# GrokImageCompression/Grok

Hardware: AMD Instinct MI355X
Metric: encode Mpixels/s (whole node), 8K RGB HTJ2K lossless (higher is better)
Workload: dtype int16x2 packed (exact: range-proven on the host, int32 fallback); 1 GPU; 8192x8192x3 8-bit RGB, 1 tile, RCT+5/3 lossless HTJ2K, 5 levels, 64x64 blocks (BASELINE metric shape); tiles_per_gpu=1, code_blocks_per_gpu=49152, packed_dwt_levels=4, generator=G2 (SURVEY.md §8d), parallelism=1 GPU, consecutive encodes pipelined (grk_amd_set_pipelining), prewarm_steps=40, input_frames_in_rotation=3

## Files before the change

### grok_amd/csrc/kernels_ht.hip

```cpp
#include <atomic>
#include <mutex>
#include "kernels.h"
#include "ht_common.h"
#include "ht_vlc_tables.h"
#define GRK_K3_STORE(p, v) __builtin_nontemporal_store((uint32_t)(v), (p))
#include <type_traits>

namespace grk_amd {

namespace {

typedef unsigned short u16x2 __attribute__((ext_vector_type(2)));
typedef int i32x2 __attribute__((ext_vector_type(2)));
typedef short i16x2 __attribute__((ext_vector_type(2)));

__device__ uint32_t g_vlc_enc[4096];
__device__ uint2 g_uvlc[64];

struct MelState {
    int run, k, acc, left;
    uint32_t pos;
    uint32_t word;
    uint32_t vec;
};
extern "C" __device__ int grk_amd_writelane(int value, int lane_select, int old) __asm("llvm.amdgcn.writelane.i32");
__device__ __forceinline__ void mel_writelane(uint32_t& vec, uint32_t word, uint32_t lane_index)
{
    vec = (uint32_t)grk_amd_writelane(__builtin_amdgcn_readfirstlane((int)word), __builtin_amdgcn_readfirstlane((int)lane_index), (int)vec);
}
struct MelPacked { uint32_t st, word, vec; uint64_t q; uint32_t qn; };
__device__ __forceinline__ void mel_drain(MelState& m, uint64_t q, uint32_t qn);
__device__ __forceinline__ MelState mel_unpack(const MelPacked& p)
{
    const uint32_t st = (uint32_t)__builtin_amdgcn_readfirstlane((int)p.st);
    MelState m;
    m.run = (int)(st & 63u); m.k = (int)((st >> 6) & 15u); m.acc = (int)((st >> 10) & 255u); m.left = (int)((st >> 18) & 15u);
    m.pos = st >> 22; m.word = (uint32_t)__builtin_amdgcn_readfirstlane((int)p.word); m.vec = p.vec;
    const uint64_t q = ((uint64_t)(uint32_t)__builtin_amdgcn_readfirstlane((int)(uint32_t)(p.q >> 32)) << 32) |
                       (uint32_t)__builtin_amdgcn_readfirstlane((int)(uint32_t)p.q);
    mel_drain(m, q, (uint32_t)__builtin_amdgcn_readfirstlane((int)p.qn));
    return m;
}
__device__ __forceinline__ void mel_pack(MelPacked& p, const MelState& m)
{
    p.st = (uint32_t)m.run | ((uint32_t)m.k << 6) | (((uint32_t)m.acc & 255u) << 10) | ((uint32_t)m.left << 18) | (m.pos << 22);
    p.word = m.word; p.vec = m.vec; p.q = 0; p.qn = 0;
}
__device__ __forceinline__ void mel_put_byte(MelState& m, uint32_t byte)
{
    if (m.pos < 252) {
        m.word |= byte << (8u * (m.pos & 3u));
        if ((m.pos & 3u) == 3u) { mel_writelane(m.vec, m.word, m.pos >> 2); m.word = 0; }
    }
    m.pos++;
}
__device__ __forceinline__ void mel_put_bit(MelState& m, uint8_t*, int v, bool)
{
    m.acc = (m.acc << 1) | v;
    if (--m.left == 0) {
        mel_put_byte(m, (uint32_t)m.acc & 0xFFu);
        m.left = (m.acc == 0xFF) ? 7 : 8;
        m.acc = 0;
    }
}
__device__ __forceinline__ void mel_put_bits(MelState& m, uint32_t v, uint32_t n)
{
    if ((int)n < m.left) { m.acc = (m.acc << n) | (int)v; m.left -= (int)n; return; }
    const uint32_t rem = n - (uint32_t)m.left;
    const uint32_t byte = (((uint32_t)m.acc << m.left) | (v >> rem)) & 0xFFu;
    mel_put_byte(m, byte);
    m.left = (byte == 0xFFu ? 7 : 8) - (int)rem;
    m.acc = (int)(v & ((1u << rem) - 1u));
}
__device__ __forceinline__ void mel_flush(MelState& m, uint8_t* buf, int lane)
{
    if (m.pos < 252 && (m.pos & 3u)) mel_writelane(m.vec, m.word, m.pos >> 2);
    reinterpret_cast<uint32_t*>(buf)[lane] = m.vec;
}

__device__ __forceinline__ void mel_event(MelState& m, uint8_t* buf, int one, bool writer)
{
    const int e = (int)((kMelE >> (4 * m.k)) & 0xF);
    if (!one) {
        if (++m.run >= (1 << e)) {
            mel_put_bit(m, buf, 1, writer);
            m.run = 0;
            if (m.k < 12) m.k++;
        }
    } else {
        mel_put_bits(m, (uint32_t)m.run, (uint32_t)e + 1u);
        m.run = 0;
        if (m.k > 0) m.k--;
    }
}

__device__ __forceinline__ void mel_drain(MelState& m, uint64_t q, uint32_t qn)
{
    while ((int)qn >= m.left) {
        qn -= (uint32_t)m.left;
        const uint32_t byte = (((uint32_t)m.acc << m.left) | ((uint32_t)(q >> qn) & ((1u << m.left) - 1u))) & 0xFFu;
        mel_put_byte(m, byte);
        m.left = byte == 0xFFu ? 7 : 8;
        m.acc = 0;
    }
    m.acc = (int)(((uint32_t)m.acc << qn) | ((uint32_t)q & ((1u << qn) - 1u)));
    m.left -= (int)qn;
}
__device__ __forceinline__ void mel_drain_packed(uint32_t& st, MelPacked& p, uint64_t& q, uint32_t& qn)
{
    MelState m;
    m.run = 0; m.k = 0; m.acc = (int)((st >> 10) & 255u); m.left = (int)((st >> 18) & 15u);
    m.pos = st >> 22; m.word = (uint32_t)__builtin_amdgcn_readfirstlane((int)p.word); m.vec = p.vec;
    mel_drain(m, q, qn);
    st = (st & 0x3FFu) | (((uint32_t)m.acc & 255u) << 10) | ((uint32_t)m.left << 18) | (m.pos << 22);
    p.word = m.word; p.vec = m.vec;
    q = 0; qn = 0;
}
__device__ __forceinline__ void mel_zeros(uint32_t& run, uint32_t& k4, uint64_t& q, uint32_t& qn, uint32_t nz)
{
    while (true) {
        const uint32_t need = (1u << ((uint32_t)(kMelE >> k4) & 0xFu)) - run;
        if (nz < need) { run += nz; break; }
        q = (q << 1) | 1u; qn += 1u;
        run = 0; k4 = min(k4 + 4u, 48u); nz -= need;
    }
}
__device__ __forceinline__ void mel_first_row(MelPacked& p, uint64_t EH, uint64_t EV)
{
    uint32_t run = 0, k4 = 0, qn = 0;
    uint64_t q = 0;
    if (!(EH & EV)) mel_zeros(run, k4, q, qn, (uint32_t)__builtin_popcountll(EH));
    else while (EH) {
        uint32_t e = (uint32_t)(kMelE >> k4) & 0xFu;
        uint32_t n, v, at, t0, t1, t2;
        asm volatile("s_ff1_i32_b64 %[at], %[EH]\n\t"
                     "s_bitset0_b64 %[EH], %[at]\n\t"
                     "s_add_i32 %[t1], %[run], 1\n\t"
                     "s_lshr_b32 %[t0], %[t1], %[e]\n\t"
                     "s_add_i32 %[t2], %[t0], -1\n\t"
                     "s_and_b32 %[t1], %[t1], %[t2]\n\t"
                     "s_lshl2_add_u32 %[t2], %[t0], %[k4]\n\t"
                     "s_min_i32 %[t2], %[t2], 48\n\t"
                     "s_add_i32 %[k4], %[k4], -4\n\t"
                     "s_max_i32 %[k4], %[k4], 0\n\t"
                     "s_add_i32 %[e], %[e], 1\n\t"
                     "s_bitcmp1_b64 %[EV], %[at]\n\t"
                     "s_cselect_b32 %[n], %[e], %[t0]\n\t"
                     "s_cselect_b32 %[v], %[run], %[t0]\n\t"
                     "s_cselect_b32 %[run], 0, %[t1]\n\t"
                     "s_cselect_b32 %[k4], %[k4], %[t2]"
                     : [EH] "+s"(EH), [run] "+s"(run), [k4] "+s"(k4), [e] "+s"(e), [n] "=&s"(n), [v] "=&s"(v), [at] "=&s"(at),
                       [t0] "=&s"(t0), [t1] "=&s"(t1), [t2] "=&s"(t2)
                     : [EV] "s"(EV)
                     : "scc");
        q = (q << n) | v; qn += n;
    }
    p.st = (p.st & ~0x3FFu) | run | (k4 << 4);
    p.q = q; p.qn = qn;
}

__device__ __forceinline__ void mel_row(MelPacked& p, uint64_t H, uint64_t V)
{
    uint32_t st = (uint32_t)__builtin_amdgcn_readfirstlane((int)p.st);
    uint32_t run = st & 63u, k4 = (st >> 4) & 0x3Cu;
    uint64_t q = ((uint64_t)(uint32_t)__builtin_amdgcn_readfirstlane((int)(uint32_t)(p.q >> 32)) << 32) |
                 (uint32_t)__builtin_amdgcn_readfirstlane((int)(uint32_t)p.q);
    uint32_t qn = (uint32_t)__builtin_amdgcn_readfirstlane((int)p.qn);
    if (__builtin_expect(qn > 40u, 0)) mel_drain_packed(st, p, q, qn);
    uint64_t ones = H & V;
    while (ones) {
        const uint32_t first = (uint32_t)__builtin_ctzll(ones);
        const uint64_t from = ~0ull << first;
        const uint32_t nz = (uint32_t)__builtin_popcountll(H & ~from);
        H &= from << 1; ones &= from << 1;
        uint32_t e = (uint32_t)(kMelE >> k4) & 0xFu;
        if (__builtin_expect(run + nz >= (1u << e), 0)) { mel_zeros(run, k4, q, qn, nz); e = (uint32_t)(kMelE >> k4) & 0xFu; }
        else run += nz;
        q = (q << (e + 1u)) | run; qn += e + 1u;
        run = 0; k4 = (uint32_t)max((int)k4 - 4, 0);
        if (__builtin_expect(qn > 40u, 0)) mel_drain_packed(st, p, q, qn);
    }
    if (H) mel_zeros(run, k4, q, qn, (uint32_t)__builtin_popcountll(H));
    p.st = (st & ~0x3FFu) | run | (k4 << 4);
    p.q = q; p.qn = qn;
}

__device__ __forceinline__ void mel_zero_run(MelState& m, uint8_t* buf, uint32_t n, bool writer)
{
    while (n) {
        const uint32_t need = (1u << ((kMelE >> (4 * m.k)) & 0xF)) - (uint32_t)m.run;
        if (n < need) { m.run += (int)n; return; }
        mel_put_bit(m, buf, 1, writer);
        m.run = 0;
        if (m.k < 12) m.k++;
        n -= need;
    }
}

__device__ __forceinline__ void or3_now(uint32_t& acc, uint32_t a, uint32_t b)
{
    asm("v_bitop3_b32 %0, %1, %2, %3 bitop3:0xfe" : "=v"(acc) : "v"(acc), "v"(a), "v"(b));
}
__device__ __forceinline__ void lds_or(uint32_t* p, uint32_t v)
{
    (void)__hip_atomic_fetch_or(p, v, __ATOMIC_RELAXED, __HIP_MEMORY_SCOPE_WORKGROUP);
}
__device__ __forceinline__ void or_bits64(uint32_t* raw, uint32_t pos, uint64_t val, uint32_t nbits)
{
    const uint32_t sh = pos & 31;
    uint32_t* w = raw + (pos >> 5);
    const uint64_t lo = val << sh;
    lds_or(w, (uint32_t)lo);
    lds_or(w + 1, (uint32_t)(lo >> 32));
    if (__ballot(sh + nbits > 64u)) lds_or(w + 2, ((uint32_t)(val >> 32) >> 1) >> (31 - sh));
}
__device__ __forceinline__ void or_bits32(uint32_t* raw, uint32_t pos, uint32_t val)
{
    const uint32_t sh = pos & 31;
    uint32_t* w = raw + (pos >> 5);
    const uint64_t lo = (uint64_t)val << sh;
    lds_or(w, (uint32_t)lo);
    lds_or(w + 1, (uint32_t)(lo >> 32));
}
__device__ __forceinline__ uint32_t get_bits(const uint32_t* raw, uint32_t pos, uint32_t n)
{
    const uint32_t w = pos >> 5, sh = pos & 31;
    uint64_t v = raw[w] | ((uint64_t)raw[w + 1] << 32);
    return (uint32_t)(v >> sh) & ((1u << n) - 1);
}

__device__ __forceinline__ uint32_t ffbh_i32(uint32_t t)
{
    uint32_t r;
    asm("v_ffbh_i32 %0, %1" : "=v"(r) : "v"(t));
    return r;
}

__device__ __forceinline__ uint32_t ffbh_u32(uint32_t t)
{
    uint32_t r;
    asm("v_ffbh_u32 %0, %1" : "=v"(r) : "v"(t));
    return r;
}
template <int B, int HALF>
__device__ __forceinline__ void ffbh_u16_to_byte(uint32_t& acc, uint32_t packed)
{
    if constexpr (B == 0) {
        if constexpr (HALF == 0) asm("v_ffbh_u32_sdwa %0, %1 dst_sel:BYTE_0 dst_unused:UNUSED_PAD src0_sel:WORD_0" : "=v"(acc) : "v"(packed));
        else asm("v_ffbh_u32_sdwa %0, %1 dst_sel:BYTE_0 dst_unused:UNUSED_PAD src0_sel:WORD_1" : "=v"(acc) : "v"(packed));
    } else if constexpr (B == 1) {
        if constexpr (HALF == 0) asm("v_ffbh_u32_sdwa %0, %1 dst_sel:BYTE_1 dst_unused:UNUSED_PRESERVE src0_sel:WORD_0" : "+v"(acc) : "v"(packed));
        else asm("v_ffbh_u32_sdwa %0, %1 dst_sel:BYTE_1 dst_unused:UNUSED_PRESERVE src0_sel:WORD_1" : "+v"(acc) : "v"(packed));
    } else if constexpr (B == 2) {
        if constexpr (HALF == 0) asm("v_ffbh_u32_sdwa %0, %1 dst_sel:BYTE_2 dst_unused:UNUSED_PRESERVE src0_sel:WORD_0" : "+v"(acc) : "v"(packed));
        else asm("v_ffbh_u32_sdwa %0, %1 dst_sel:BYTE_2 dst_unused:UNUSED_PRESERVE src0_sel:WORD_1" : "+v"(acc) : "v"(packed));
    } else {
        if constexpr (HALF == 0) asm("v_ffbh_u32_sdwa %0, %1 dst_sel:BYTE_3 dst_unused:UNUSED_PRESERVE src0_sel:WORD_0" : "+v"(acc) : "v"(packed));
        else asm("v_ffbh_u32_sdwa %0, %1 dst_sel:BYTE_3 dst_unused:UNUSED_PRESERVE src0_sel:WORD_1" : "+v"(acc) : "v"(packed));
    }
}
template <int B>
__device__ __forceinline__ void ffbh_i32_to_byte(uint32_t& acc, uint32_t t)
{
    if constexpr (B == 0) asm("v_ffbh_i32_sdwa %0, %1 dst_sel:BYTE_0 dst_unused:UNUSED_PAD src0_sel:DWORD" : "=v"(acc) : "v"(t));
    else if constexpr (B == 1) asm("v_ffbh_i32_sdwa %0, %1 dst_sel:BYTE_1 dst_unused:UNUSED_PRESERVE src0_sel:DWORD" : "+v"(acc) : "v"(t));
    else if constexpr (B == 2) asm("v_ffbh_i32_sdwa %0, %1 dst_sel:BYTE_2 dst_unused:UNUSED_PRESERVE src0_sel:DWORD" : "+v"(acc) : "v"(t));
    else asm("v_ffbh_i32_sdwa %0, %1 dst_sel:BYTE_3 dst_unused:UNUSED_PRESERVE src0_sel:DWORD" : "+v"(acc) : "v"(t));
}
__device__ __forceinline__ uint32_t min_of_bytes(uint32_t c)
{
    uint32_t m1, m2;
    asm("v_min_u32_sdwa %0, %1, %1 dst_sel:DWORD dst_unused:UNUSED_PAD src0_sel:BYTE_0 src1_sel:BYTE_1" : "=v"(m1) : "v"(c));
    asm("v_min_u32_sdwa %0, %1, %1 dst_sel:DWORD dst_unused:UNUSED_PAD src0_sel:BYTE_2 src1_sel:BYTE_3" : "=v"(m2) : "v"(c));
    return min(m1, m2);
}
template <int TT>
__device__ __forceinline__ uint32_t bitop3(uint32_t a, uint32_t b, uint32_t c)
{
    return (uint32_t)__builtin_amdgcn_bitop3_b32((int)a, (int)b, (int)c, TT);
}
__device__ __forceinline__ uint32_t pk_min_u16(uint32_t a, uint32_t b)
{
    uint32_t r;
    asm("v_pk_min_u16 %0, %1, %2" : "=v"(r) : "v"(a), "s"(b));
    return r;
}
__device__ __forceinline__ uint32_t pk_lshr15_u16(uint32_t a)
{
    uint32_t r;
    asm("v_pk_lshrrev_b16 %0, 15, %1 op_sel_hi:[0,1]" : "=v"(r) : "v"(a));
    return r;
}
__device__ __forceinline__ uint32_t pk_sub_u16(uint32_t a, uint32_t b)
{
    uint32_t r;
    asm("v_pk_sub_u16 %0, %1, %2" : "=v"(r) : "v"(a), "v"(b));
    return r;
}
__device__ __forceinline__ uint32_t sign_mask(uint32_t a)
{
    uint32_t r;
    asm("v_ashrrev_i32 %0, 31, %1" : "=v"(r) : "v"(a));
    return r;
}
__device__ __forceinline__ uint32_t pk_mul_lo_u16(uint32_t a, uint32_t b)
{
    uint32_t r;
// ... 311 lines not shown
            stage1(it + 2, sE, n2); stage2(it + 1, sO);
            stage1(it + 3, sO, n3); stage2(it + 2, sE);
            stage1(it + 4, sE, n0); stage2(it + 3, sO);
        }
        stage1(it + 1, sO, n1); stage2(it, sE);
        stage1(it + 2, sE, n2); stage2(it + 1, sO);
        stage1(it + 3, sO, n3); stage2(it + 2, sE);
        stage1_last(it + 4, sE, n0); stage2(it + 3, sO);
        stage1_last(it + 5, sO, n1); stage2(it + 4, sE);
        stage1_last(it + 6, sE, n2); stage2(it + 5, sO);
        stage1_last(it + 7, sO, n3); stage2(it + 6, sE);
        stage2(it + 7, sO);
    } else {
        for (uint32_t it = 0; it < itn; it += 4) {
            if (it + 1 < itn) stage1(it + 1, sO, n1);
            stage2(it, sE);
            if (it + 1 < itn) { if (it + 2 < itn) stage1(it + 2, sE, n2); stage2(it + 1, sO); }
            if (it + 2 < itn) { if (it + 3 < itn) stage1(it + 3, sO, n3); stage2(it + 2, sE); }
            if (it + 3 < itn) { if (it + 4 < itn) stage1(it + 4, sE, n0); stage2(it + 3, sO); }
        }
        asm volatile("" : : "v"(n0[0]), "v"(n0[1]), "v"(n0[2]), "v"(n0[3]), "v"(n1[0]), "v"(n1[1]), "v"(n1[2]), "v"(n1[3]),
                            "v"(n2[0]), "v"(n2[1]), "v"(n2[2]), "v"(n2[3]), "v"(n3[0]), "v"(n3[1]), "v"(n3[2]), "v"(n3[3]));
    }
    };

    auto phase_a2 = [&]() {
        constexpr bool PK = H16;
        constexpr int NW = PK ? 4 : 8;
        const uint32_t rr = (uint32_t)lane >> 4, cc = (uint32_t)lane & 15u;
        const uint32_t c0m = cc == 0 ? 0xFFFFFFFFu : 0u, c15m = cc == 15 ? 0xFFFFFFFFu : 0u;
        const uint32_t oddm = (rr & 1u) ? 0xFFFFFFFFu : 0u, row0m = rr == 0 ? 0xFFFFFFFFu : 0u;
        const uint32_t lane_off2 = 2u * rr * stride_b + 4u * cc * EB;
        typedef int i32x4 __attribute__((ext_vector_type(4)));

        auto fetch2 = [&](uint32_t it, int32_t (&r)[NW]) {
            const uint32_t o0 = lane_off2 + it * (8u * stride_b), o1 = o0 + stride_b;
            if constexpr (PK) {
                const i32x2 q0 = __builtin_nontemporal_load(reinterpret_cast<const i32x2*>(srcb + o0));
                const i32x2 q1 = __builtin_nontemporal_load(reinterpret_cast<const i32x2*>(srcb + o1));
                r[0] = q0.x; r[1] = q1.x; r[2] = q0.y; r[3] = q1.y;
            } else {
                const i32x4 q0 = __builtin_nontemporal_load(reinterpret_cast<const i32x4*>(srcb + o0));
                const i32x4 q1 = __builtin_nontemporal_load(reinterpret_cast<const i32x4*>(srcb + o1));
                r[0] = q0.x; r[2] = q0.y; r[1] = q1.x; r[3] = q1.y;
                r[4] = q0.z; r[6] = q0.w; r[5] = q1.z; r[7] = q1.w;
            }
        };
        int32_t n0[NW], n1[NW], n2[NW], n3[NW];
        fetch2(0, n0); fetch2(1, n1); fetch2(2, n2); fetch2(3, n3);

        struct Stage1 {
            uint32_t vv[2][PK ? 2 : 4];
            uint32_t SM[2], U[2], u[2], tuple[2];
            uint2 ue[2];
            uint64_t H[2], V[2];
        };
        uint32_t Aprev = 0xFFFFFFFFu;

        auto analyse = [&](const int32_t* sm, uint32_t (&vv)[PK ? 2 : 4], uint32_t& C) {
            if constexpr (PK) {
                const int32_t nw0 = sm[0], nw1 = sm[1];
                const i16x2 w0 = __builtin_bit_cast(i16x2, nw0), w1 = __builtin_bit_cast(i16x2, nw1);
                const u16x2 p0 = __builtin_bit_cast(u16x2, __builtin_elementwise_max(w0, -w0));
                const u16x2 p1 = __builtin_bit_cast(u16x2, __builtin_elementwise_max(w1, -w1));
                or3_now(ovf, __builtin_bit_cast(uint32_t, p0), __builtin_bit_cast(uint32_t, p1));
                const u16x2 one2 = {1, 1};
                const uint32_t t0 = __builtin_bit_cast(uint32_t, __builtin_elementwise_sub_sat(p0 + p0, one2));
                const uint32_t t1 = __builtin_bit_cast(uint32_t, __builtin_elementwise_sub_sat(p1 + p1, one2));
                ffbh_u16_to_byte<0, 0>(C, t0); ffbh_u16_to_byte<1, 0>(C, t1);
                ffbh_u16_to_byte<2, 1>(C, t0); ffbh_u16_to_byte<3, 1>(C, t1);
                vv[0] = pk_sub_u16(t0, pk_lshr15_u16(~(uint32_t)nw0));
                vv[1] = pk_sub_u16(t1, pk_lshr15_u16(~(uint32_t)nw1));
            } else {
                uint32_t t[4];
#pragma unroll
                for (int i = 0; i < 4; ++i) {
                    uint32_t mag;
                    if constexpr (IRREV) {
                        const float cf = __int_as_float(sm[i]);
                        const float q = __fmul_rn(fabsf(cf), inv_step);
                        mag = min((uint32_t)q, lim);
                    } else {
                        mag = (uint32_t)max(sm[i], -sm[i]);
                    }
                    ovf |= mag;
                    t[i] = (mag << 1) - 1u;
                    vv[i] = t[i] - 1u + ((uint32_t)sm[i] >> 31);
                }
                ffbh_i32_to_byte<0>(C, t[0]); ffbh_i32_to_byte<1>(C, t[1]);
                ffbh_i32_to_byte<2>(C, t[2]); ffbh_i32_to_byte<3>(C, t[3]);
            }
        };

        auto stage1r = [&](uint32_t it, Stage1& o, int32_t (&nbuf)[NW], auto refill_c) {
            uint32_t C[2];
            analyse(nbuf, o.vv[0], C[0]);
            analyse(nbuf + NW / 2, o.vv[1], C[1]);
            uint32_t N[2], rho[2], rho2[2], cm[2], emax[2];
#pragma unroll
            for (int q = 0; q < 2; ++q) {
                N[q] = bitop3<0x30>(0x01010101u, C[q] >> 7, 0u);
                rho[q] = __builtin_amdgcn_udot4(N[q], 0x08040201u, 0u, false);
                rho2[q] = __builtin_amdgcn_udot4(N[q], 0x20100804u, 0u, false);
                cm[q] = min_of_bytes(C[q]);
                emax[q] = 32u - min(cm[q], 32u);
            }
            const uint32_t Bp = __builtin_amdgcn_perm(C[1], C[0], 0x07050301u);
            const auto s16 = __builtin_amdgcn_permlane16_swap(Bp, Bp, false, false);
            const uint32_t A1 = (uint32_t)s16[1];
            const auto s32 = __builtin_amdgcn_permlane32_swap(Aprev, A1, false, false);
            const uint32_t tsel = bitop3<0xE4>((uint32_t)s32[1], (uint32_t)s32[0], row0m);
            const uint32_t Y = bitop3<0xE4>((uint32_t)s16[0], tsel, oddm);
            Aprev = A1;
            const uint32_t Yl = dpp0<0x138, 0xF>(Y) | c0m;
            const uint32_t Yr = dpp0<0x130, 0xF>(Y) | c15m;
            const uint32_t rhoBl = dpp0<0x138, 0xF>(rho[1]) & ~c0m;
            const uint32_t W[2] = {__builtin_amdgcn_alignbit(Y, Yl, 24), __builtin_amdgcn_alignbit(Yr, Y, 8)};
            const uint32_t rl[2] = {rhoBl, rho[0]};
            bool cq0[2];
#pragma unroll
            for (int q = 0; q < 2; ++q) {
                const uint32_t m4 = min_of_bytes(W[q]);
                const int kap_e = 31 - (int)m4;
                const uint32_t gmask = sign_mask(0xFEE80000u << (15u - rho[q]));
                const uint32_t kappa = (uint32_t)max(1, kap_e & (int)gmask);
                const uint32_t F = W[q] & (W[q] >> 8);
                uint32_t coff = bitop3<0xEA>(F << 3, 0x400u, 0x2000u);
                coff = bitop3<0xEA>(F >> 11, 0x1000u, coff);
                coff = bitop3<0xEA>((rl[q] & 0xCu) + 0x7FCu, 0x800u, coff);
                cq0[q] = (coff & 0x1C00u) == 0x1400u;
                if (it == 0) {
                    const uint32_t cq_first = (rl[q] >> 1) | (rl[q] & 1u);
                    coff = rr ? coff : cq_first << 10;
                    cq0[q] = rr ? cq0[q] : cq_first == 0u;
                }
                const uint32_t U = max(emax[q], kappa);
                const uint32_t u = U - kappa;
                const uint32_t X = C[q] - __builtin_amdgcn_perm(cm[q], cm[q], 0u);
                const uint32_t Yz = (X & 0x1F1F1F1Fu) + 0x7F7F7F7Fu;
                const uint32_t e4 = __builtin_amdgcn_udot4(bitop3<0x30>(0x01010101u, Yz >> 7, 0u), 0x20100804u, 0u, false);
                const uint32_t um = sign_mask(0u - u);
                const uint32_t off = ((rho2[q] << 4) | coff) | bitop3<0x80>(e4, rho2[q], um);
                o.tuple[q] = *reinterpret_cast<const uint32_t*>(vtab + off);
                o.SM[q] = N[q] * 255u; o.U[q] = U; o.u[q] = u;
                if (it != 0) o.ue[q] = uvlc_l[u];
            }
            o.H[0] = __ballot(cq0[0]); o.V[0] = o.H[0] & __ballot(rho[0] != 0);
            o.H[1] = __ballot(cq0[1]); o.V[1] = o.H[1] & __ballot(rho[1] != 0);
            if constexpr (decltype(refill_c)::value) {
                __builtin_amdgcn_sched_barrier(0);
                fetch2(it + 4u, nbuf);
            }
        };
        auto stage1 = [&](uint32_t it, Stage1& o, int32_t (&nbuf)[NW]) { stage1r(it, o, nbuf, std::true_type{}); };
        auto stage1_last = [&](uint32_t it, Stage1& o, int32_t (&nbuf)[NW]) { stage1r(it, o, nbuf, std::false_type{}); };

        auto stage2 = [&](uint32_t it, const Stage1& s) {
            uint32_t vm[2][4], M4[2], m1[2], m2[2], m3[2], m01[2], m23[2], qlen[2];
#pragma unroll
            for (int q = 0; q < 2; ++q) {
                M4[q] = (__builtin_amdgcn_perm(s.U[q], s.U[q], 0u) - (s.tuple[q] & 0x01010101u)) & s.SM[q];
                qlen[q] = __builtin_amdgcn_udot4(M4[q], 0x01010101u, 0u, false);
                m01[q] = __builtin_amdgcn_udot4(M4[q], 0x00000101u, 0u, false);
                m23[q] = qlen[q] - m01[q];
                m1[q] = M4[q] >> 8; m2[q] = M4[q] >> 16; m3[q] = M4[q] >> 24;
                if constexpr (PK) {
                    vm[q][0] = __builtin_amdgcn_ubfe(s.vv[q][0], 0u, M4[q]); vm[q][2] = __builtin_amdgcn_ubfe(s.vv[q][0], 16u, m2[q]);
                    vm[q][1] = __builtin_amdgcn_ubfe(s.vv[q][1], 0u, m1[q]); vm[q][3] = __builtin_amdgcn_ubfe(s.vv[q][1], 16u, m3[q]);
                } else {
                    vm[q][0] = __builtin_amdgcn_ubfe(s.vv[q][0], 0u, M4[q]); vm[q][2] = __builtin_amdgcn_ubfe(s.vv[q][2], 0u, m2[q]);
                    vm[q][1] = __builtin_amdgcn_ubfe(s.vv[q][1], 0u, m1[q]); vm[q][3] = __builtin_amdgcn_ubfe(s.vv[q][3], 0u, m3[q]);
                }
            }
            const uint32_t ms_len = qlen[0] + qlen[1];

            uint32_t uiA = s.u[0], uiB = s.u[1];
            bool xev = false, xv = false;
            if (it == 0) {
                const bool first = rr == 0;
                const uint32_t uA = s.u[0], uB = s.u[1];
                const bool both = first && uA > 2 && uB > 2;
                uiA = both ? uA - 2 : uA;
                uiB = both ? uB - 2 : uB;
                uiB = (first && uA > 2 && uB > 0 && uB <= 2) ? 32u + uB : uiB;
                xev = first && uA > 0 && uB > 0;
                xv = xev && min(uA, uB) > 2;
            }
            const uint2 ueA = it == 0 ? uvlc_l[uiA] : s.ue[0], ueB = it == 0 ? uvlc_l[uiB] : s.ue[1];
            const uint32_t AA = (s.tuple[0] >> 25) | ueA.x, AB = (s.tuple[1] >> 25) | ueB.x;
            const uint32_t LA = ((s.tuple[0] >> 4) & 7u) | ueA.y, LB = ((s.tuple[1] >> 4) & 7u) | ueB.y;
            const uint32_t S = LA + LB;
            const uint32_t lenA = LA & 0xFFu, slen = S & 0xFFu;
            const uint32_t o_preB = slen + ((LA >> 8) & 0xFFu);
            const uint32_t o_sufA = slen + ((S >> 8) & 0xFFu);
            const uint32_t o_sufB = o_sufA + (LA >> 16);
            const uint32_t cl = o_sufA + (S >> 16);
            const uint32_t wv = (AA & 0xFFu) | ((AB & 0xFFu) << lenA) | (((AA >> 8) & 0xFFu) << slen) | (((AB >> 8) & 0xFFu) << o_preB) |
                                ((AA >> 16) << o_sufA) | ((AB >> 16) << o_sufB);

            const uint32_t packed = ms_len | (cl << 16);
            const uint32_t incl = wave_incl_scan(packed);
            const uint32_t tot = (uint32_t)__builtin_amdgcn_readlane((int)incl, 63);
            const uint32_t mpos = ms_bits + ((incl - packed) & 0xFFFFu);
            const uint32_t vpos = vlc_bits + (incl >> 16) - cl;
            ms_bits += tot & 0xFFFFu;
            vlc_bits += tot >> 16;
            if (((L.ms_cap_bits - ms_bits) | (L.vlc_cap_bits - vlc_bits)) >> 31) { lds_full = true; return; }

            if (ms_len != 0u) {
                if (!__ballot(max(qlen[0], qlen[1]) > 32u)) {
                    const uint32_t qa = (vm[0][0] | (vm[0][1] << (M4[0] & 31u))) | ((vm[0][2] | (vm[0][3] << (m2[0] & 31u))) << (m01[0] & 31u));
                    const uint32_t qb = (vm[1][0] | (vm[1][1] << (M4[1] & 31u))) | ((vm[1][2] | (vm[1][3] << (m2[1] & 31u))) << (m01[1] & 31u));
                    or_bits64(ms_raw, mpos, (uint64_t)qa | ((uint64_t)qb << qlen[0]), ms_len);
                } else {
#pragma unroll
                    for (int q = 0; q < 2; ++q) {
                        const uint32_t at = q ? mpos + qlen[0] : mpos;
                        if (narrow || !__ballot(max(m01[q], m23[q]) > 32u)) {
                            const uint32_t v01 = vm[q][0] | (vm[q][1] << (M4[q] & 31u));
                            const uint32_t v23 = vm[q][2] | (vm[q][3] << (m2[q] & 31u));
                            or_bits64(ms_raw, at, (uint64_t)v01 | ((uint64_t)v23 << m01[q]), qlen[q]);
                        } else {
                            or_bits64(ms_raw, at, (uint64_t)vm[q][0] | ((uint64_t)vm[q][1] << (M4[q] & 0xFFu)), m01[q]);
                            or_bits64(ms_raw, at + m01[q], (uint64_t)vm[q][2] | ((uint64_t)vm[q][3] << (m2[q] & 0xFFu)), m23[q]);
                        }
                    }
                }
            }
            if (cl != 0u) or_bits32(vlc_raw, vpos, wv);

            uint64_t HA = s.H[0], VA = s.V[0], HB = s.H[1], VB = s.V[1];
            if (it != 0 && !(HA | HB)) return;
            if (it == 0) {
                const uint32_t lo = (uint32_t)lane & 31u;
                const uint32_t fl = (((uint32_t)HA >> lo) & 1u) | ((((uint32_t)HB >> lo) & 1u) << 1) | (xev ? 4u : 0u) |
                                    ((((uint32_t)VA >> lo) & 1u) << 3) | ((((uint32_t)VB >> lo) & 1u) << 4) | (xv ? 32u : 0u);
                const uint32_t third = ((uint32_t)lane * 43u) >> 7;
                const uint32_t g = (uint32_t)__builtin_amdgcn_ds_bpermute((int)(4u * third), (int)fl) >> ((uint32_t)lane - 3u * third);
                const bool in_row = lane < 48;
                const uint64_t EH = __ballot(in_row && (g & 1u)), EV = EH & __ballot((g & 8u) != 0u);
                mel_first_row(melp, EH, EV);
                HA &= ~0xFFFFull; HB &= ~0xFFFFull;
            }
            if (!(HA | HB)) return;
            MelState mel = mel_unpack(melp);
            while (HA | HB) {
                const uint64_t oa = HA & VA, ob = HB & VB;
                if (!(oa | ob)) {
                    mel_zero_run(mel, mel_buf, (uint32_t)(__builtin_popcountll(HA) + __builtin_popcountll(HB)), lane == 0);
                    break;
                }
                const uint32_t la = oa ? (uint32_t)__builtin_ctzll(oa) : 64u, lb = ob ? (uint32_t)__builtin_ctzll(ob) : 64u;
                const bool a_first = (int)(la - lb) <= 0;
                const uint32_t ln = a_first ? la : lb;
                const uint64_t bit = 1ull << ln, below = bit - 1;
                const uint64_t ma = a_first ? below : (below | bit);
                mel_zero_run(mel, mel_buf, (uint32_t)(__builtin_popcountll(HA & ma) + __builtin_popcountll(HB & below)), lane == 0);
                mel_event(mel, mel_buf, 1, lane == 0);
                HA &= ~(below | bit);
                HB &= a_first ? ~below : ~(below | bit);
            }
            mel_pack(melp, mel);
        };

        Stage1 sE, sO;
        stage1(0, sE, n0);
        stage1(1, sO, n1); stage2(0, sE);
        stage1(2, sE, n2); stage2(1, sO);
        stage1(3, sO, n3); stage2(2, sE);
        stage1_last(4, sE, n0); stage2(3, sO);
        stage1_last(5, sO, n1); stage2(4, sE);
        stage1_last(6, sE, n2); stage2(5, sO);
        stage1_last(7, sO, n3); stage2(6, sE);
        stage2(7, sO);
    };
    if constexpr (H16) {
        if (full && ((bd.px | a.stride) & 3u) == 0) phase_a2(); else phase_a(std::false_type{});
    } else {
        if (full) phase_a(std::true_type{}); else phase_a(std::false_type{});
    }
    if (lds_full) {
        if (lane == 0) {
            const unsigned long long at = __hip_atomic_fetch_add(a.alloc + 2 + class_id, 1ull, __ATOMIC_RELAXED, __HIP_MEMORY_SCOPE_AGENT);
            a.ovf_list[a.ovf_base + at] = tile * a.sel_count + li;
        }
        return;
    }
    if constexpr (H16) ovf = (ovf & 0xFFFFu) | (ovf >> 16);
    if (!IRREV && __ballot((ovf >> (kmax + 1)) != 0)) {
        if (lane == 0) atomicOr(reinterpret_cast<unsigned int*>(a.alloc), 2u);
    }
    __syncthreads();

    MelState mel = mel_unpack(melp);
    const uint32_t len_ub = (ms_bits + ms_bits / 15u) / 8u + (vlc_bits + vlc_bits / 15u) / 8u + mel.pos + 8u;
    unsigned long long base_off = 0;
    if (lane == 0) base_off = arena_alloc(a.alloc, gid & a.region_mask, len_ub, a.chunk_units);

    uint8_t* const vst = reinterpret_cast<uint8_t*>(uvlc_l);
    typedef uint32_t u32_lds_any __attribute__((aligned(1)));
    uint32_t nv, vposr;
    {
        uint32_t s = 0, i = 0, prev = 0xFFu << 24;
        while (true) {
            const uint32_t avail = (vlc_bits - s) >> 3;
            if (avail == 0) break;
            const uint32_t start = s + 32u * (uint32_t)lane;
            const uint32_t sw = start >> 5;
            const uint32_t win = __builtin_amdgcn_alignbit(vlc_raw[sw + 1], vlc_raw[sw], start);
            const uint32_t before = (uint32_t)__builtin_amdgcn_update_dpp((int)prev, (int)win, 0x138, 0xF, 0xF, false);
            const uint32_t pw = __builtin_amdgcn_alignbit(win, before, 24);
            const uint32_t e = (win & 0x7F7F7F7Fu) + 0x01010101u;
            uint32_t z = bitop3<0x80>(pw >> 3, (pw >> 2) | (pw >> 1) | pw, e >> 3) & 0x10101010u;
            const uint32_t lane4s = 4u * (uint32_t)lane;
            uint32_t nb = 4;
            if (avail < 256u) {
                nb = min(avail - min(avail, lane4s), 4u);
                z &= nb >= 4u ? 0xFFFFFFFFu : (1u << (8u * nb)) - 1u;
            }
            const uint64_t ballot = __ballot(z != 0);
            const uint32_t F = ballot ? (uint32_t)__ffsll((long long)ballot) - 1u : 64u;
            if ((uint32_t)lane < F) {
                if (nb == 4u) *reinterpret_cast<u32_lds_any*>(vst + i + lane4s) = win;
                else {
#pragma unroll 1
                    for (uint32_t k = 0; k < nb; ++k) vst[i + lane4s + k] = (uint8_t)(win >> (8u * k));
                }
            }
            if (!ballot) {
                const uint32_t n = min(avail, 256u);
                const uint32_t lw = (uint32_t)__builtin_amdgcn_readlane((int)win, (int)((n - 1u) >> 2));
                prev = (lw >> (8u * ((n - 1u) & 3u))) << 24;
                s += 8u * n; i += n;
                continue;
            }
            const uint32_t zF = (uint32_t)__builtin_amdgcn_readlane((int)z, (int)F);
            const uint32_t winF = (uint32_t)__builtin_amdgcn_readlane((int)win, (int)F);
            const uint32_t b = (uint32_t)(__ffs((int)zF) - 1) >> 3;
            i += 4u * F;
            if ((uint32_t)lane <= b)
                vst[i + lane] = (uint8_t)((winF >> (8u * lane)) & ((uint32_t)lane == b ? 0x7Fu : 0xFFu));
            s += 32u * F + 8u * b + 7u; i += b + 1u; prev = 0x7Fu << 24;
        }
        if (vlc_bits - s == 7u && (prev >> 24) > 0x8Fu &&
            (uint32_t)__builtin_amdgcn_readfirstlane((int)get_bits(vlc_raw, s, 7u)) == 0x7Fu) {
            if (lane == 0) vst[i] = 0x7Fu;
            i += 1u; s += 7u;
        }
        nv = i; vposr = s;
    }
    const uint32_t vused = vlc_bits - vposr;
    const uint32_t vacc = vused ? get_bits(vlc_raw, vposr, vused) : 0;

    if (mel.run > 0) mel_put_bit(mel, mel_buf, 1, lane == 0);
    uint32_t vextra = 0;
    {
        const int macc = mel.acc << mel.left;
        const int mel_mask = (0xFF << mel.left) & 0xFF;
        const int vlc_mask = 0xFF >> (8 - (int)vused);
        if ((mel_mask | vlc_mask) != 0) {
            const int fuse = macc | (int)vacc;
            if ((((fuse ^ macc) & mel_mask) | ((fuse ^ (int)vacc) & vlc_mask)) == 0 && fuse != 0xFF && nv >= 1) {
                mel_put_byte(mel, (uint32_t)fuse & 0xFFu);
            } else {
                mel_put_byte(mel, (uint32_t)macc & 0xFFu);
                vextra = 1;
            }
        }
    }
    mel_flush(mel, mel_buf, lane);
    const uint32_t mel_len = mel.pos;
    const uint32_t vcount = nv + vextra;
    const uint32_t scup = mel_len + vcount + 1;

    base_off = ((unsigned long long)(uint32_t)__builtin_amdgcn_readfirstlane((int)(uint32_t)(base_off >> 32)) << 32) |
               (uint32_t)__builtin_amdgcn_readfirstlane((int)(uint32_t)base_off);
    if (base_off + len_ub > a.arena_bytes) {
        if (lane == 0) { a.lengths[gid] = 0; a.offsets[gid] = base_off; atomicOr(reinterpret_cast<unsigned int*>(a.alloc), 1u); }
        return;
    }
    uint8_t* const out = a.arena + base_off;
    typedef uint32_t u32_any __attribute__((aligned(1)));
    const uint32_t lane32 = 32u * (uint32_t)lane, lane4 = 4u * (uint32_t)lane;

    uint32_t ms_len;
    {
        uint32_t s = 0, j = 0;
        bool done = false;
        while (s + 8u <= ms_bits) {
            const uint32_t avail = (ms_bits - s) >> 3;
            const uint32_t start = s + lane32;
            const uint32_t sw = start >> 5;
            const uint32_t win = __builtin_amdgcn_alignbit(ms_raw[sw + 1], ms_raw[sw], start);
            uint32_t z = bitop3<0x80>(~win - 0x01010101u, win, 0x80808080u);
            uint32_t nb = 4;
            if (avail < 256u) {
                nb = min(avail - min(avail, lane4), 4u);
                z &= nb >= 4u ? 0xFFFFFFFFu : (1u << (8u * nb)) - 1u;
            }
            const uint64_t ballot = __ballot(z != 0);
            if (!ballot) {
                if (avail >= 256u) {
                    GRK_K3_STORE(reinterpret_cast<u32_any*>(out + j + lane4), win);
                    s += 2048u; j += 256u;
                    continue;
                }
                if (nb == 4u) GRK_K3_STORE(reinterpret_cast<u32_any*>(out + j + lane4), win);
                else {
#pragma unroll 1
                    for (uint32_t k = 0; k < nb; ++k) out[j + lane4 + k] = (uint8_t)(win >> (8u * k));
                }
                s += 8u * avail; j += avail;
                continue;
            }
            const uint32_t F = (uint32_t)__ffsll((long long)ballot) - 1u;
            const uint32_t zF = (uint32_t)__builtin_amdgcn_readlane((int)z, (int)F);
            const uint32_t winF = (uint32_t)__builtin_amdgcn_readlane((int)win, (int)F);
            const uint32_t b = (uint32_t)(__ffs((int)zF) - 1) >> 3;
            if ((uint32_t)lane < F) GRK_K3_STORE(reinterpret_cast<u32_any*>(out + j + lane4), win);
            const uint32_t p7 = s + 32u * F + 8u * (b + 1u);
            uint32_t winN;
            if (F < 63u) winN = (uint32_t)__builtin_amdgcn_readlane((int)win, (int)(F + 1u));
            else {
                const uint32_t sn = s + 2048u;
                winN = (uint32_t)__builtin_amdgcn_readfirstlane((int)__builtin_amdgcn_alignbit(ms_raw[(sn >> 5) + 1u], ms_raw[sn >> 5], sn));
            }
            const uint64_t tail = (((uint64_t)winN << 32) | winF) >> (8u * (b + 1u));
            j += 4u * F;
            if (p7 == ms_bits) {
                if ((uint32_t)lane < b) out[j + lane] = (uint8_t)(winF >> (8u * lane));
                ms_len = j + b; done = true;
                break;
            }
            if ((uint32_t)lane <= b) out[j + lane] = (uint8_t)(winF >> (8u * lane));
            j += b + 1u;
            if (p7 + 7u > ms_bits) {
                const uint32_t rem = ms_bits - p7;
                const uint32_t fin = ((uint32_t)tail & ((1u << rem) - 1u)) | ((((1u << (7u - rem)) - 1u) << rem) & 0x7Fu);
                if (lane == 0) out[j] = (uint8_t)fin;
                ms_len = j + 1u; done = true;
                break;
            }
            const uint32_t b7 = (uint32_t)tail & 0x7Fu;
            if (lane == 0) out[j] = (uint8_t)b7;
            j += 1u;
            s = p7 + 7u;
            if (s + 15u <= ms_bits && ((uint32_t)(tail >> 7) & 0xFFu) == 0xFFu)
            while (s + 15u <= ms_bits) {
                const uint32_t two = (uint32_t)__builtin_amdgcn_readfirstlane((int)get_bits(ms_raw, s, 15u));
                if ((two & 0xFFu) != 0xFFu) break;
                if (lane == 0) { out[j] = 0xFFu; out[j + 1u] = (uint8_t)(two >> 8); }
                j += 2u; s += 15u;
            }
        }
        if (!done) {
            const uint32_t rem = ms_bits - s;
            if (rem) {
                const uint32_t fin = get_bits(ms_raw, s, rem) | ((((1u << (8u - rem)) - 1u) << rem) & 0xFFu);
                if (fin != 0xFFu) {
                    if (lane == 0) out[j] = (uint8_t)fin;
                    j += 1u;
                }
            }
            ms_len = j;
        }
    }
    const uint32_t total = ms_len + mel_len + vcount + 1;
    if (lane == 0) { a.lengths[gid] = total; a.offsets[gid] = base_off; }
    if (total > len_ub) {
        if (lane == 0) atomicOr(reinterpret_cast<unsigned int*>(a.alloc), 1u);
        return;
    }
    __syncthreads();
#pragma unroll 1
    for (uint32_t i = lane; i < mel_len; i += 64) out[ms_len + i] = mel_buf[i < 250 ? i : 249];

    {
        uint8_t* const last = out + total - 2;
#pragma unroll 1
        for (uint32_t k = 4u * (uint32_t)lane; k < nv; k += 256u) {
            uint32_t word = *reinterpret_cast<const uint32_t*>(vst + k);
            if (k == 0) word = (word & ~0xFu) | (scup & 0xFu);
            const uint32_t n = min(nv - k, 4u);
            if (n == 4u) GRK_K3_STORE(reinterpret_cast<u32_any*>(last - 3 - (int)k), __builtin_bswap32(word));
            else {
#pragma unroll 1
                for (uint32_t t = 0; t < n; ++t) *(last - (int)(k + t)) = (uint8_t)(word >> (8u * t));
            }
        }
    }
    if (lane == 0) {
        if (vextra) out[total - 2 - nv] = (uint8_t)(nv == 0 ? ((vacc & 0xF0) | (scup & 0xF)) : vacc);
        out[total - 1] = (uint8_t)(scup >> 4);
    }
}

template <bool IRREV, bool H16, bool ROOM>
__global__ __launch_bounds__(64) void ht_encode_kernel(HtArgs a, HtLds L, uint32_t class_id)
{
    if constexpr (ROOM) asm volatile("" ::: "v103");
    ht_encode_block<IRREV, H16>(a, blockIdx.x % a.sel_count, blockIdx.x / a.sel_count, L, class_id);
}


template <bool IRREV, bool H16>
__global__ __launch_bounds__(64) void ht_encode_fallback_kernel(HtArgs a, HtLds L, uint32_t class_id)
{
    const uint32_t count = (uint32_t)a.alloc[2 + class_id];
    for (uint32_t i = blockIdx.x; i < count; i += gridDim.x) {
        const uint32_t id = a.ovf_list[a.ovf_base + i];
        ht_encode_block<IRREV, H16>(a, id % a.sel_count, id / a.sel_count, L, class_id);
        __syncthreads();
    }
}

}

static std::atomic<bool> g_tables_ready[16];
static std::mutex g_tables_mu;
static const uint32_t* g_vlc_tab_dev[16] = {nullptr};

static hipError_t upload_tables()
{
    static uint32_t enc[4096];
    auto entry = [](uint32_t t) {
        const uint32_t ek = t & 15u;
        return ((t >> 8) << 25) | (((t >> 4) & 7u) << 4) | (ek & 1u) | (((ek >> 1) & 1u) << 8) | (((ek >> 2) & 1u) << 16) | ((ek >> 3) << 24);
    };
    for (uint32_t i = 0; i < 2048; ++i) {
        enc[i] = entry(HT_VLC_ENC0[i]);
        const uint32_t ctx = i >> 8, n_w = ctx & 1u, rl = (ctx >> 1) & 1u, n_e = (ctx >> 2) & 1u;
        const uint32_t c_q = (n_w ? 0u : 1u) | (rl << 1) | ((n_e ? 0u : 1u) << 2);
        enc[2048 + i] = entry(HT_VLC_ENC1[(c_q << 8) | (i & 0xFFu)]);
    }
    static uint2 uv[64];
    for (uint32_t u = 0; u < 64; ++u) {
        uint32_t pre = 0, pl = 0, suf = 0, sl = 0;
        if (u < 32) {
            if (u <= 2)      { pre = u; pl = u; }
            else if (u <= 4) { pre = 4; pl = 3; suf = u - 3; sl = 1; }
            else             { pre = 0; pl = 3; suf = u - 5; sl = 5; }
        } else if (u == 33 || u == 34) { pre = u - 33; pl = 1; }
        uv[u].x = (pre << 8) | (suf << 16);
        uv[u].y = (pl << 8) | (sl << 16);
    }
    hipError_t e = hipMemcpyToSymbol(HIP_SYMBOL(g_vlc_enc), enc, sizeof(enc), 0, hipMemcpyHostToDevice);
    if (e != hipSuccess) return e;
    return hipMemcpyToSymbol(HIP_SYMBOL(g_uvlc), uv, sizeof(uv), 0, hipMemcpyHostToDevice);
}

static hipError_t ensure_tables(const uint32_t** tab = nullptr)
{
    int dev = 0;
    hipError_t e = hipGetDevice(&dev);
    if (e != hipSuccess) return e;
    if (dev < 0 || dev >= 16) return hipErrorInvalidDevice;
    if (!g_tables_ready[dev].load(std::memory_order_acquire)) {
        std::lock_guard<std::mutex> lk(g_tables_mu);
        if (!g_tables_ready[dev].load(std::memory_order_relaxed)) {
            e = upload_tables();
            if (e != hipSuccess) return e;
            void* p = nullptr;
            e = hipGetSymbolAddress(&p, HIP_SYMBOL(g_vlc_enc));
            if (e != hipSuccess) return e;
            g_vlc_tab_dev[dev] = static_cast<const uint32_t*>(p);
            g_tables_ready[dev].store(true, std::memory_order_release);
        }
    }
    if (tab) *tab = g_vlc_tab_dev[dev];
    return hipSuccess;
}

hipError_t launch_ht_alloc_init(const HtArgs& a, hipStream_t s)
{
    hipError_t e = ensure_tables();
    if (e != hipSuccess) return e;
    hipLaunchKernelGGL(ht_alloc_init_kernel, dim3(1), dim3(64), 0, s, a.alloc, a.chunk_units);
    return hipGetLastError();
}

hipError_t launch_ht_classes(const HtArgs& a, uint32_t first, uint32_t last, hipStream_t s)
{
    const uint32_t* vlc_tab = nullptr;
    hipError_t e = ensure_tables(&vlc_tab);
    if (e != hipSuccess) return e;
    for (uint32_t k = first; k < last && k < a.num_classes; ++k) {
        const HtClass& c = a.classes[k];
        if (c.count == 0) continue;
        const HtClassLds lds = plan_ht_lds(c.max_samples, c.max_quads, c.max_kmax, c.cap_kmax, a.irreversible != 0, a.ovf_list != nullptr);
        auto kernel_arg = [](const HtLdsPlan& p) { return HtLds{p.ms_words, p.vlc_words, p.ms_cap_bits, p.vlc_cap_bits, p.stage_bytes}; };
        const bool use_cap = lds.use_cap;
        const HtLds full = kernel_arg(lds.full), L = kernel_arg(use_cap ? lds.cap : lds.full);
        const size_t shmem_full = lds.full.bytes, shmem = use_cap ? lds.cap.bytes : lds.full.bytes;
        HtArgs b = a;
        b.sel = c.sel; b.sel_count = c.count;
        b.ovf_base = c.ovf_base;
        b.vlc_tab = vlc_tab;
        const uint32_t grid = c.count * a.ntiles;
#define GRK_HT(KERNEL, G, SH, LL)                                                                                                   \
        do {                                                                                                                        \
            if (a.h16 && !a.irreversible) hipLaunchKernelGGL((KERNEL<false, true>), dim3(G), dim3(64), SH, s, b, LL, k);         \
            else if (a.irreversible)      hipLaunchKernelGGL((KERNEL<true, false>), dim3(G), dim3(64), SH, s, b, LL, k);          \
            else                          hipLaunchKernelGGL((KERNEL<false, false>), dim3(G), dim3(64), SH, s, b, LL, k);         \
        } while (0)
        if (a.h16 && !a.irreversible && a.room) hipLaunchKernelGGL((ht_encode_kernel<false, true, true>), dim3(grid), dim3(64), shmem, s, b, L, k);
        else if (a.h16 && !a.irreversible)      hipLaunchKernelGGL((ht_encode_kernel<false, true, false>), dim3(grid), dim3(64), shmem, s, b, L, k);
        else if (a.irreversible)                hipLaunchKernelGGL((ht_encode_kernel<true, false, false>), dim3(grid), dim3(64), shmem, s, b, L, k);
        else                                    hipLaunchKernelGGL((ht_encode_kernel<false, false, false>), dim3(grid), dim3(64), shmem, s, b, L, k);
        if (use_cap) GRK_HT(ht_encode_fallback_kernel, std::min<uint32_t>(grid, 1024u), shmem_full, full);
#undef GRK_HT
    }
    return hipGetLastError();
}

hipError_t launch_ht_encode(const HtArgs& a, hipStream_t s)
{
    hipError_t e = launch_ht_alloc_init(a, s);
    if (e != hipSuccess) return e;
    return launch_ht_classes(a, 0, a.num_classes, s);
}

}
```

Baseline: 195,000 Mpixels/s.

## Resolve multiple bit-stuffing events per window pass in HT MagSgn and VLC packing

Adds a wave-wide window pass that handles up to 16 bit-stuffing events inside one 2048-bit window. It shifts the lanes above each event by recomputing their words with per-lane alignbit offsets, instead of restarting the whole window after every event. This targets the serial cost of the stuffing loop in the MagSgn and VLC byte emitters, where each event used to trigger a fresh window load, ballot and readlanes. In exchange the per-iteration arithmetic is heavier, there is a restart flag that falls back to the old path, and the shift-and-carry logic is complex enough to risk subtle errors in the lossless bitstream.

```diff
diff --git a/grok_amd/csrc/ht_stuff_lanes.h b/grok_amd/csrc/ht_stuff_lanes.h
--- /dev/null
+++ b/grok_amd/csrc/ht_stuff_lanes.h
@@ -0,0 +1,111 @@
+#pragma once
+#include <stdint.h>
+
+namespace hsl {
+
+constexpr uint32_t kMaxEvents = 16;
+constexpr uint32_t kWindowBits = 2048;
+constexpr uint32_t kInteriorBits = kWindowBits + 32;
+
+#if defined(__HIP_DEVICE_COMPILE__) || defined(__HIPCC__)
+#define HSL_FN __device__ __forceinline__
+typedef uint32_t V;
+typedef bool P;
+HSL_FN V lane_ids() { return (uint32_t)__lane_id(); }
+HSL_FN P gt(V a, uint32_t s) { return a > s; }
+HSL_FN P eq(V a, uint32_t s) { return a == s; }
+HSL_FN P nz(V a) { return a != 0; }
+HSL_FN V sel(P p, V a, V b) { return p ? a : b; }
+HSL_FN uint64_t ballot(P p) { return __ballot(p); }
+HSL_FN uint32_t readlane(V v, uint32_t l) { return (uint32_t)__builtin_amdgcn_readlane((int)v, (int)l); }
+HSL_FN V shift_up(V v, uint32_t first) { return (uint32_t)__builtin_amdgcn_update_dpp((int)first, (int)v, 0x138, 0xF, 0xF, false); }
+HSL_FN V alignbit(V hi, V lo, V sh) { return __builtin_amdgcn_alignbit(hi, lo, sh); }
+HSL_FN uint32_t ctz64(uint64_t v) { return (uint32_t)__ffsll((long long)v) - 1u; }
+HSL_FN uint32_t ctz32(uint32_t v) { return (uint32_t)__ffs((int)v) - 1u; }
+#else
+#define HSL_FN static inline
+struct V {
+    uint32_t l[64];
+    V() : l{} {}
+    V(uint32_t s) { for (int i = 0; i < 64; ++i) l[i] = s; }
+};
+struct P { uint64_t m; };
+#define HSL_BINOP(op) \
+    HSL_FN V operator op(const V& a, const V& b) { V r; for (int i = 0; i < 64; ++i) r.l[i] = a.l[i] op b.l[i]; return r; }
+HSL_BINOP(+) HSL_BINOP(-) HSL_BINOP(&) HSL_BINOP(|)
+#undef HSL_BINOP
+HSL_FN V operator>>(const V& a, uint32_t s) { V r; for (int i = 0; i < 64; ++i) r.l[i] = a.l[i] >> s; return r; }
+HSL_FN V operator<<(const V& a, uint32_t s) { V r; for (int i = 0; i < 64; ++i) r.l[i] = a.l[i] << s; return r; }
+HSL_FN V lane_ids() { V r; for (int i = 0; i < 64; ++i) r.l[i] = (uint32_t)i; return r; }
+HSL_FN P gt(const V& a, uint32_t s) { P p{0}; for (int i = 0; i < 64; ++i) p.m |= (uint64_t)(a.l[i] > s) << i; return p; }
+HSL_FN P eq(const V& a, uint32_t s) { P p{0}; for (int i = 0; i < 64; ++i) p.m |= (uint64_t)(a.l[i] == s) << i; return p; }
+HSL_FN P nz(const V& a) { P p{0}; for (int i = 0; i < 64; ++i) p.m |= (uint64_t)(a.l[i] != 0) << i; return p; }
+HSL_FN V sel(P p, const V& a, const V& b) { V r; for (int i = 0; i < 64; ++i) r.l[i] = (p.m >> i) & 1 ? a.l[i] : b.l[i]; return r; }
+HSL_FN uint64_t ballot(P p) { return p.m; }
+HSL_FN uint32_t readlane(const V& v, uint32_t l) { return v.l[l & 63u]; }
+HSL_FN V shift_up(const V& v, uint32_t first) { V r; r.l[0] = first; for (int i = 1; i < 64; ++i) r.l[i] = v.l[i - 1]; return r; }
+HSL_FN V alignbit(const V& hi, const V& lo, const V& sh)
+{
+    V r;
+    for (int i = 0; i < 64; ++i) r.l[i] = (uint32_t)((((uint64_t)hi.l[i] << 32) | lo.l[i]) >> (sh.l[i] & 31u));
+    return r;
+}
+HSL_FN uint32_t ctz64(uint64_t v) { return (uint32_t)__builtin_ctzll(v); }
+HSL_FN uint32_t ctz32(uint32_t v) { return (uint32_t)__builtin_ctz(v); }
+#endif
+
+template <bool VLC>
+HSL_FN V event_flags(const V& cur, uint32_t prev)
+{
+    const V e = (cur & V(0x7F7F7F7Fu)) + V(0x01010101u);
+    if constexpr (!VLC) {
+        (void)prev;
+        return e & cur & V(0x80808080u);
+    } else {
+        const V pw = alignbit(cur, shift_up(cur, prev), V(24u));
+        return (pw >> 3) & ((pw >> 2) | (pw >> 1) | pw) & (e >> 3) & V(0x10101010u);
+    }
+}
+
+struct PassResult {
+    uint32_t lanes;
+    uint32_t extra;
+    uint32_t bits;
+    uint32_t events;
+};
+
+template <bool VLC>
+HSL_FN PassResult window_pass(const V& w0, const V& lane, uint32_t prev, V& cur)
+{
+    const V wp = shift_up(w0, 0u);
+    V nk(0u);
+    V valid(0xFFFFFFFFu);
+    cur = w0;
+    PassResult r{64u, 0u, kWindowBits, 0u};
+    uint32_t slot0 = 64u;
+    while (true) {
+        const V fl = event_flags<VLC>(cur, prev) & valid;
+        const uint64_t bal = ballot(nz(fl));
+        if (!bal) { r.bits = kWindowBits - r.events; return r; }
+        const uint32_t F = ctz64(bal);
+        const uint32_t b = ctz32(readlane(fl, F)) >> 3;
+        const uint32_t tgt = VLC ? F : F + (b == 3u);
+        if (r.events == kMaxEvents || tgt > 63u) {
+            r.lanes = F;
+            r.extra = !VLC && slot0 == F;
+            r.events = r.extra - readlane(nk, F);
+            r.bits = 32u * F + 8u * r.extra - r.events;
+            return r;
+        }
+        const uint32_t at = VLC ? 8u * b + 7u : (8u * b + 15u) & 31u;
+        if (!VLC && b == 3u) slot0 = tgt;
+        const P above = gt(lane, tgt);
+        nk = sel(above, nk - V(1u), nk);
+        cur = sel(above, alignbit(w0, wp, nk), cur);
+        cur = sel(eq(lane, tgt), cur + (cur & V(0xFFFFFFFFu << at)), cur);
+        valid = sel(gt(lane, F), V(0xFFFFFFFFu), sel(eq(lane, F), V(b == 3u ? 0u : 0xFFFFFF00u << (8u * b)), V(0u)));
+        ++r.events;
+    }
+}
+
+}
diff --git a/grok_amd/csrc/kernels_ht.hip b/grok_amd/csrc/kernels_ht.hip
--- a/grok_amd/csrc/kernels_ht.hip
+++ b/grok_amd/csrc/kernels_ht.hip
@@ -3,6 +3,7 @@
 #include "kernels.h"
 #include "ht_common.h"
 #include "ht_vlc_tables.h"
+#include "ht_stuff_lanes.h"
 #define GRK_K3_STORE(p, v) __builtin_nontemporal_store((uint32_t)(v), (p))
 #include <type_traits>
 
@@ -920,6 +921,7 @@
     uint32_t nv, vposr;
     {
         uint32_t s = 0, i = 0, prev = 0xFFu << 24;
+        bool restart = false;
         while (true) {
             const uint32_t avail = (vlc_bits - s) >> 3;
             if (avail == 0) break;
@@ -937,6 +939,15 @@
                 z &= nb >= 4u ? 0xFFFFFFFFu : (1u << (8u * nb)) - 1u;
             }
             const uint64_t ballot = __ballot(z != 0);
+            if (ballot && !restart && s + hsl::kInteriorBits <= vlc_bits) {
+                uint32_t cur;
+                const hsl::PassResult r = hsl::window_pass<true>(win, (uint32_t)lane, prev, cur);
+                if ((uint32_t)lane < r.lanes) *reinterpret_cast<u32_lds_any*>(vst + i + lane4s) = cur;
+                prev = (uint32_t)__builtin_amdgcn_readlane((int)cur, (int)(r.lanes - 1u)) & 0xFF000000u;
+                s += r.bits; i += 4u * r.lanes;
+                restart = r.lanes < 64u;
+                continue;
+            }
             const uint32_t F = ballot ? (uint32_t)__ffsll((long long)ballot) - 1u : 64u;
             if ((uint32_t)lane < F) {
                 if (nb == 4u) *reinterpret_cast<u32_lds_any*>(vst + i + lane4s) = win;
@@ -952,6 +963,7 @@
                 s += 8u * n; i += n;
                 continue;
             }
+            restart = false;
             const uint32_t zF = (uint32_t)__builtin_amdgcn_readlane((int)z, (int)F);
             const uint32_t winF = (uint32_t)__builtin_amdgcn_readlane((int)win, (int)F);
             const uint32_t b = (uint32_t)(__ffs((int)zF) - 1) >> 3;
@@ -1004,7 +1016,7 @@
     uint32_t ms_len;
     {
         uint32_t s = 0, j = 0;
-        bool done = false;
+        bool done = false, restart = false;
         while (s + 8u <= ms_bits) {
             const uint32_t avail = (ms_bits - s) >> 3;
             const uint32_t start = s + lane32;
@@ -1031,6 +1043,16 @@
                 s += 8u * avail; j += avail;
                 continue;
             }
+            if (!restart && s + hsl::kInteriorBits <= ms_bits) {
+                uint32_t cur;
+                const hsl::PassResult r = hsl::window_pass<false>(win, (uint32_t)lane, 0u, cur);
+                if ((uint32_t)lane < r.lanes) GRK_K3_STORE(reinterpret_cast<u32_any*>(out + j + lane4), cur);
+                if (r.extra && (uint32_t)lane == r.lanes) out[j + lane4] = (uint8_t)cur;
+                s += r.bits; j += 4u * r.lanes + r.extra;
+                restart = r.lanes < 64u;
+                continue;
+            }
+            restart = false;
             const uint32_t F = (uint32_t)__ffsll((long long)ballot) - 1u;
             const uint32_t zF = (uint32_t)__builtin_amdgcn_readlane((int)z, (int)F);
             const uint32_t winF = (uint32_t)__builtin_amdgcn_readlane((int)win, (int)F);
```

New measurement: 195,200 Mpixels/s, median of 2. No clear change (+0.1%).
